# kutieme/avenir

Measured on AMD Instinct MI355X. Metric: naive_bayes_train_rows_per_s, higher is better.
Workload: dtype row-packed categorical records (11-bit records, lossless)/int64 counts (exact); 1 GPU; model=NaiveBayes(resource/churn.json: 5 categorical features, 2 classes), global_batch=1073741824, rows_per_gpu=1073741824, parallelism=dp1

## Files before the change

### avenir_amd/csrc/bindings.cpp

```cpp
#include <atomic>
#include <cstdlib>
#include <condition_variable>
#include <cstring>
#include <functional>
#include <chrono>
#include <limits>
#include <map>
#include <memory>
#include <mutex>
#include <thread>
#include <unistd.h>
#include <sys/stat.h>
#include <sys/mman.h>
#include <fcntl.h>
#include <torch/extension.h>
#include <ATen/hip/impl/HIPGuardImplMasqueradingAsCUDA.h>
#include <ATen/hip/impl/HIPStreamMasqueradingAsCUDA.h>

#include "avenir_kernels.h"
#include "avenir_host.h"

namespace {

using DevGuard = c10::hip::HIPGuardMasqueradingAsCUDA;
// ... 139 lines not shown
    TORCH_CHECK(widths[k] >= 1 && widths[k] <= 8 && shifts[k] >= 0 && shifts[k] + widths[k] <= B,
                "packed field outside the record");
    sh[k] = (int)shifts[k];
    wd[k] = (int)widths[k];
  }
  TORCH_CHECK(n_classes >= 1 && n_classes <= 2, "1 or 2 classes");
  CHECK_DEV(bins); CHECK_DTYPE(bins, at::kInt);
  CHECK_DEV(offs); CHECK_DTYPE(offs, at::kInt);
  TORCH_CHECK(bins.numel() == F && offs.numel() == F, "bins / offs must have F entries");
  TORCH_CHECK((int64_t)bins_host.size() == F && (int64_t)offs_host.size() == F, "bins_host / offs_host: F entries");
  for (int64_t k = 0; k < F; ++k)
    TORCH_CHECK(offs_host[k] >= 0 && bins_host[k] >= 1 && offs_host[k] + bins_host[k] <= total_bins,
                "feature bins outside the table");
  CHECK_DEV(out); CHECK_DTYPE(out, at::kLong);
  TORCH_CHECK(out.numel() == n_classes * total_bins, "out must be [C * TB]");
  DevGuard g(dense.device());
  avk::class_histogram_dense(reinterpret_cast<const uint32_t*>(dense.data_ptr<int>()), n, (int)B, sh.data(), wd.data(),
                             (int)F, (int)label_shift, (int)label_width, bins.data_ptr<int>(), offs.data_ptr<int>(),
                             (int)total_bins, (int)n_classes, count_labels ? 1 : 0,
                             reinterpret_cast<unsigned long long*>(out.data_ptr<int64_t>()), cur_stream(dense));
}

static std::vector<int> radix_ints(const std::vector<int64_t>& v, int64_t F, const char* what) {
  TORCH_CHECK((int64_t)v.size() == F, what, ": F entries");
  std::vector<int> r(F);
  for (int64_t k = 0; k < F; ++k) {
    TORCH_CHECK(v[k] >= 0 && v[k] < (int64_t(1) << 30), what, " out of range");
    r[k] = (int)v[k];
  }
  return r;
}

std::vector<int64_t> radix_shape(std::vector<int64_t> radices, int64_t class_radix, int64_t n_classes,
                                 int64_t total_bins) {
  TORCH_CHECK(class_radix >= 1 && class_radix <= 3 && n_classes >= 1 && n_classes <= 2 && total_bins >= 0 &&
                  total_bins < (int64_t(1) << 24), "bad class radix / classes / table width");
  int64_t J = class_radix;
  for (int64_t r : radices) {
    TORCH_CHECK(r >= 1 && r <= 9, "radix out of range");
    J *= r;
    TORCH_CHECK(J <= (int64_t(1) << 40), "too many joint states");
  }
  return {J, (int64_t)avk::radix_bits(J), (int64_t)avk::radix_replicas(J, (int)n_classes, (int)total_bins)};
}

at::Tensor pack_radix(const at::Tensor& words, int64_t n, int64_t B, std::vector<int64_t> shifts,
                      std::vector<int64_t> widths, std::vector<int64_t> radices, std::vector<int64_t> bins_host,
                      int64_t label_shift, int64_t class_radix, int64_t n_classes) {
  CHECK_DEV(words);
  CHECK_DTYPE(words, at::kShort);
  TORCH_CHECK(words.dim() == 1 && n >= 0 && n <= words.numel(), "words must be [>= n]");
  TORCH_CHECK(B >= 4 && B <= 15, "4..15 bits per record");
  const int64_t F = (int64_t)shifts.size();
  TORCH_CHECK(F >= 1 && F <= 8, "1..8 packed fields");
  const auto sh = radix_ints(shifts, F, "shifts"), wd = radix_ints(widths, F, "widths");
  const auto rad = radix_ints(radices, F, "radices"), hb = radix_ints(bins_host, F, "bins");
  auto dense = at::zeros({std::max<int64_t>(1, avk::dense_words(n, (int)B))}, words.options().dtype(at::kInt));
  DevGuard g(words.device());
  avk::pack_radix(reinterpret_cast<const uint16_t*>(words.data_ptr()), n, (int)B, sh.data(), wd.data(), rad.data(),
                  hb.data(), (int)F, (int)label_shift, (int)class_radix, (int)n_classes,
                  reinterpret_cast<uint32_t*>(dense.data_ptr<int>()), cur_stream(words));
  return dense;
}

void class_histogram_radix(const at::Tensor& dense, int64_t n, int64_t B, std::vector<int64_t> radices,
                           std::vector<int64_t> bins_host, std::vector<int64_t> offs_host, int64_t class_radix,
                           int64_t total_bins, int64_t n_classes, at::Tensor& out, bool count_labels) {
  CHECK_DEV(dense);
  CHECK_DTYPE(dense, at::kInt);
  TORCH_CHECK(B >= 4 && B <= 15 && n >= 0 && dense.numel() >= avk::dense_words(n, (int)B), "radix stream too short");
  const int64_t F = (int64_t)radices.size();
  TORCH_CHECK(F >= 1 && F <= 8, "1..8 packed fields");
  const auto rad = radix_ints(radices, F, "radices"), hb = radix_ints(bins_host, F, "bins");
  const auto ho = radix_ints(offs_host, F, "offs");
  TORCH_CHECK(n_classes >= 1 && n_classes <= 2, "1 or 2 classes");
  TORCH_CHECK(total_bins >= 1 && total_bins < (int64_t(1) << 24), "bad table width");
  CHECK_DEV(out); CHECK_DTYPE(out, at::kLong);
  TORCH_CHECK(out.numel() == n_classes * total_bins, "out must be [C * TB]");
  DevGuard g(dense.device());
  avk::class_histogram_radix(reinterpret_cast<const uint32_t*>(dense.data_ptr<int>()), n, (int)B, rad.data(), hb.data(),
                             ho.data(), (int)F, (int)class_radix, (int)total_bins, (int)n_classes,
                             count_labels ? 1 : 0, reinterpret_cast<unsigned long long*>(out.data_ptr<int64_t>()),
                             cur_stream(dense));
}

void pair_histogram(const at::Tensor& codes, int64_t n, const c10::optional<at::Tensor>& labels,
                    const at::Tensor& bins, const at::Tensor& pairs, const at::Tensor& poff,
                    int64_t max_tab, int64_t n_classes, at::Tensor& out) {
  CHECK_DEV(codes);
  CHECK_DTYPE(codes, at::kByte);
  TORCH_CHECK(codes.dim() == 2 && n <= codes.size(1), "codes must be [F, ld>=n]");
  CHECK_DEV(bins);
  CHECK_DTYPE(bins, at::kInt);
  CHECK_DEV(pairs);
  CHECK_DTYPE(pairs, at::kInt);
  CHECK_DEV(poff);
  CHECK_DTYPE(poff, at::kLong);
  CHECK_DEV(out);
  CHECK_DTYPE(out, at::kLong);
  TORCH_CHECK(pairs.dim() == 2 && pairs.size(1) == 2, "pairs must be [P,2]");
  TORCH_CHECK(poff.numel() == pairs.size(0), "poff must be [P]");
  const uint8_t* lab = nullptr;
  if (labels.has_value() && labels->defined()) {
    CHECK_DEV((*labels));
    CHECK_DTYPE((*labels), at::kByte);
    TORCH_CHECK(labels->numel() >= n, "labels shorter than n");
    lab = labels->data_ptr<uint8_t>();
  }
  DevGuard g(codes.device());
  avk::pair_histogram(codes.data_ptr<uint8_t>(), codes.size(1), n, lab, bins.data_ptr<int>(),
                      pairs.data_ptr<int>(), reinterpret_cast<const long long*>(poff.data_ptr<int64_t>()), (int)pairs.size(0),
                      (int)max_tab, (int)n_classes,
                      reinterpret_cast<unsigned long long*>(out.data_ptr<int64_t>()),
                      cur_stream(codes));
}

void bigram_histogram(const at::Tensor& states, const c10::optional<at::Tensor>& labels,
                      int64_t n_classes, int64_t S, at::Tensor& out) {
  CHECK_DEV(states);
  CHECK_DTYPE(states, at::kShort);
  TORCH_CHECK(states.dim() == 2, "states must be [N, L]");
  CHECK_DEV(out);
  CHECK_DTYPE(out, at::kLong);
  TORCH_CHECK(out.numel() == n_classes * S * S, "out must be [C*S*S]");
  TORCH_CHECK(S >= 1 && S <= 32767, "bad S");
  const uint8_t* lab = nullptr;
  if (labels.has_value() && labels->defined()) {
    CHECK_DEV((*labels));
    CHECK_DTYPE((*labels), at::kByte);
    TORCH_CHECK(labels->numel() >= states.size(0), "labels shorter than N");
    lab = labels->data_ptr<uint8_t>();
  }
  DevGuard g(states.device());
  avk::bigram_histogram(states.data_ptr<int16_t>(), states.size(0), (int)states.size(1), lab,
                        (int)n_classes, (int)S,
                        reinterpret_cast<unsigned long long*>(out.data_ptr<int64_t>()),
                        cur_stream(states));
}

at::Tensor class_moments(const at::Tensor& x, int64_t n, const c10::optional<at::Tensor>& labels,
                         int64_t n_classes) {
  CHECK_DEV(x);
  CHECK_DTYPE(x, at::kFloat);
  TORCH_CHECK(x.dim() == 2 && n <= x.size(1), "x must be [F, ld>=n]");
  const uint8_t* lab = nullptr;
  if (labels.has_value() && labels->defined()) {
    CHECK_DEV((*labels));
    CHECK_DTYPE((*labels), at::kByte);
    TORCH_CHECK(labels->numel() >= n, "labels shorter than n");
    lab = labels->data_ptr<uint8_t>();
  }
  const int64_t F = x.size(0);
  DevGuard g(x.device());
  auto opts = x.options().dtype(at::kDouble);
  auto out = at::zeros({n_classes, F, 3}, opts);
  const int nb = avk::moments_blocks(n);
  auto part = at::empty({nb, n_classes, F, 3}, opts);
  avk::class_moments(x.data_ptr<float>(), x.size(1), n, (int)F, lab, (int)n_classes,
                     part.data_ptr<double>(), nb, out.data_ptr<double>(), cur_stream(x));
  return out;
}

void nb_predict(const at::Tensor& codes, int64_t n, const at::Tensor& offs, const at::Tensor& logp,
                const c10::optional<at::Tensor>& logfp, const c10::optional<at::Tensor>& x,
                const c10::optional<at::Tensor>& gmean, const c10::optional<at::Tensor>& ginvstd,
                const c10::optional<at::Tensor>& glognorm, const c10::optional<at::Tensor>& pmean,
// ... 3555 lines not shown
                    training ? gates.data_ptr<float>() : nullptr, training ? hx.data_ptr<float>() : nullptr,
                    cur_stream(wfrag));
  if (training) return {hseq, cseq, gates, hx};
  return {hseq, cseq};
}

std::vector<at::Tensor> lstm_backward_f32(const at::Tensor& dhseq, const at::Tensor& gates, const at::Tensor& cseq,
                                          const c10::optional<at::Tensor>& c0, const c10::optional<at::Tensor>& dhn,
                                          const c10::optional<at::Tensor>& dcn, const at::Tensor& wfragT, int64_t H) {
  const int64_t KS = lstm_ks(H), HP = 32 * KS;
  for (const at::Tensor* t : std::initializer_list<const at::Tensor*>{&dhseq, &gates, &cseq, &wfragT}) {
    CHECK_DEV((*t));
    CHECK_DTYPE((*t), at::kFloat);
    TORCH_CHECK(t->is_contiguous() && aligned(*t, 16), "LSTM backward inputs must be contiguous and 16-byte aligned");
  }
  TORCH_CHECK(dhseq.dim() == 3 && dhseq.size(2) == H, "dhseq must be [B, T, H]");
  const int64_t B = dhseq.size(0), T = dhseq.size(1);
  TORCH_CHECK(cseq.dim() == 3 && cseq.size(0) == B && cseq.size(1) == T && cseq.size(2) == HP,
              "cseq must be [B, T, HP]");
  TORCH_CHECK(gates.dim() == 3 && gates.size(0) == B && gates.size(1) == T && gates.size(2) == 4 * HP,
              "gates must be [B, T, 4HP]");
  TORCH_CHECK(wfragT.numel() == 2 * KS * HP * 64, "wfragT must be [NW, HP, 64]");
  check_opt_f32(c0, B * H, "c0");
  check_opt_f32(dhn, B * H, "dhn");
  check_opt_f32(dcn, B * H, "dcn");
  DevGuard g(dhseq.device());
  auto dz = at::empty({B, T, 4 * H}, dhseq.options());
  auto dh0 = at::empty({B, H}, dhseq.options()), dc0 = at::empty({B, H}, dhseq.options());
  avk::lstm_bwd_f32(dhseq.data_ptr<float>(), gates.data_ptr<float>(), cseq.data_ptr<float>(), ptr_or_null<float>(c0),
                    ptr_or_null<float>(dhn), ptr_or_null<float>(dcn), wfragT.data_ptr<float>(), (int)B, (int)T, (int)H,
                    (int)KS, dz.data_ptr<float>(), dh0.data_ptr<float>(), dc0.data_ptr<float>(), cur_stream(dhseq));
  return {dz, dh0, dc0};
}

std::vector<at::Tensor> lstm_backward(const at::Tensor& dhseq, const at::Tensor& gates, const at::Tensor& cseq,
                                      const c10::optional<at::Tensor>& c0, const c10::optional<at::Tensor>& dhn,
                                      const c10::optional<at::Tensor>& dcn, const at::Tensor& wfragT, int64_t H) {
  const int64_t KS = lstm_ks(H), HP = 32 * KS;
  for (const at::Tensor* t : std::initializer_list<const at::Tensor*>{&dhseq, &gates, &cseq}) {
    CHECK_DEV((*t));
    CHECK_DTYPE((*t), t == &gates ? at::kBFloat16 : at::kFloat);
    TORCH_CHECK(aligned(*t, 16), "LSTM backward inputs must be 16-byte aligned");
  }
  TORCH_CHECK(dhseq.dim() == 3 && dhseq.size(2) == H, "dhseq must be [B, T, H]");
  const int64_t B = dhseq.size(0), T = dhseq.size(1);
  TORCH_CHECK(cseq.dim() == 3 && cseq.size(0) == B && cseq.size(1) == T && cseq.size(2) == HP,
              "cseq must be [B, T, HP]");
  TORCH_CHECK(gates.dim() == 3 && gates.size(0) == B && gates.size(1) == T && gates.size(2) == 4 * HP,
              "gates must be [B, T, 4HP]");
  CHECK_DEV(wfragT);
  CHECK_DTYPE(wfragT, at::kBFloat16);
  TORCH_CHECK(wfragT.numel() == 2 * KS * 4 * KS * 64 * 8, "wfragT must be [NW, 4KS, 64, 8]");
  TORCH_CHECK(aligned(wfragT, 16), "wfragT must be 16-byte aligned");
  check_opt_f32(c0, B * H, "c0");
  check_opt_f32(dhn, B * H, "dhn");
  check_opt_f32(dcn, B * H, "dcn");
  DevGuard g(dhseq.device());
  auto dz = at::empty({B, T, 4 * HP}, dhseq.options().dtype(at::kBFloat16));
  auto dh0 = at::empty({B, H}, dhseq.options()), dc0 = at::empty({B, H}, dhseq.options());
  const int RT = avk::lstm_row_tiles(B, (int)KS);
  avk::lstm_bwd(dhseq.data_ptr<float>(), reinterpret_cast<const unsigned short*>(gates.data_ptr()),
                cseq.data_ptr<float>(), ptr_or_null<float>(c0), ptr_or_null<float>(dhn), ptr_or_null<float>(dcn),
                wfragT.data_ptr(), (int)B, (int)T, (int)H, (int)KS, RT,
                reinterpret_cast<unsigned short*>(dz.data_ptr()), dh0.data_ptr<float>(), dc0.data_ptr<float>(),
                cur_stream(dhseq));
  return {dz, dh0, dc0};
}

}

void register_comm(py::module_& m);

PYBIND11_MODULE(_C, m) {
  register_comm(m);
  m.doc() = "avenir_amd native kernels (HIP/CDNA4 gfx950) and host runtime";
  m.def("class_histogram", &class_histogram);
  m.def("pair_histogram", &pair_histogram);
  m.def("class_histogram_rowpacked", &class_histogram_rowpacked);
  m.def("pack_dense", &pack_dense);
  m.def("class_histogram_dense", &class_histogram_dense);
  m.def("radix_shape", &radix_shape);
  m.def("pack_radix", &pack_radix);
  m.def("class_histogram_radix", &class_histogram_radix);
  m.def("bigram_histogram", &bigram_histogram);
  m.def("class_moments", &class_moments);
  m.def("nb_predict", &nb_predict);
  m.def("nb_predict_wide", &nb_predict_wide);
  m.def("node_histogram", &node_histogram, py::arg("codes"), py::arg("n"), py::arg("labels"), py::arg("node"),
        py::arg("weight"), py::arg("bins"), py::arg("offs"), py::arg("total_bins"), py::arg("n_classes"),
        py::arg("n_nodes"), py::arg("hist"), py::arg("node_rows") = py::none());
  m.def("node_grad_histogram", &node_grad_histogram, py::arg("codes"), py::arg("n"), py::arg("node"), py::arg("g"),
        py::arg("h"), py::arg("bins"), py::arg("offs"), py::arg("total_bins"), py::arg("n_nodes"), py::arg("out"),
        py::arg("even_only") = false, py::arg("tot_slot") = -1, py::arg("scale") = 65536.0);
  m.def("gbt_grad", &gbt_grad);
  m.def("gbt_split", &gbt_split);
  m.def("rank_avg", &rank_avg);
  m.def("tfidf_csr", &tfidf_csr);
  m.def("mixed_knn", &mixed_knn);
  m.def("pagerank", &pagerank);
  m.def("pagerank_multi", &pagerank_multi);
  m.def("sgns_hot_replicas", &avk::sgns_hot_replicas);
  m.def("sgns_step", &sgns_step, py::arg("Win"), py::arg("Wout"), py::arg("gIn"), py::arg("gOut"), py::arg("cIn"),
        py::arg("cOut"), py::arg("centre"), py::arg("context"), py::arg("aprob"), py::arg("alias"), py::arg("neg"),
        py::arg("lr"), py::arg("mean_in"), py::arg("seed"), py::arg("step"), py::arg("hot") = py::none(),
        py::arg("gOutHot") = py::none(), py::arg("gInHot") = py::none(), py::arg("cIn_next") = py::none(),
        py::arg("cOut_next") = py::none());
  m.def("kendall_pairs", &kendall_pairs);
  m.def("inversion_count", &inversion_count);
  m.def("resample_uniform", &resample_uniform);
  m.def("smote", &smote);
  m.def("gbt_assign", &gbt_assign);
  m.def("tree_assign", &tree_assign);
  m.def("tree_predict", &tree_predict);
  m.def("knn_topk", &knn_topk, py::arg("Q"), py::arg("R"), py::arg("k"), py::arg("q_base"), py::arg("r_base"),
        py::arg("exclude_self"), py::arg("splits"), py::arg("metric"), py::arg("p"), py::arg("prec") = -1);
  m.def("knn_mode", &avk::knn_mode);
  m.def("knn_vote", &knn_vote);
  m.def("cluster_accumulate", &cluster_accumulate);
  m.def("viterbi", &viterbi);
  m.def("viterbi_chunks", &viterbi_chunks);
  m.def("viterbi_backtrack", &viterbi_backtrack);
  m.def("markov_logodds", &markov_logodds);
  m.def("itemset_support", &itemset_support);
  m.def("build_bitsets", &build_bitsets);
  m.def("bandit_select", &bandit_select);
  m.def("sample", &sample);
  m.def("philox_normal", [](int64_t seed, int64_t offset, int64_t index_base, int64_t n, bool pairs,
                            c10::optional<at::Device> device) {
    TORCH_CHECK(n >= 0 && index_base >= 0, "philox_normal: n, index_base >= 0");
    if (device.has_value() && device->is_cuda()) {
      auto out = pairs ? at::empty({n, 2}, at::TensorOptions().dtype(at::kDouble).device(*device))
                       : at::empty({n}, at::TensorOptions().dtype(at::kDouble).device(*device));
      DevGuard g(*device);
      avk::philox_normal((unsigned long long)seed, (unsigned long long)offset, (unsigned long long)index_base, n,
                         out.data_ptr<double>(), pairs ? 1 : 0, cur_stream(out));
      return out;
    }
    auto out = pairs ? at::empty({n, 2}, at::TensorOptions().dtype(at::kDouble))
                     : at::empty({n}, at::TensorOptions().dtype(at::kDouble));
    {
      py::gil_scoped_release nogil;
      const unsigned hc = std::thread::hardware_concurrency();
      avh::philox_normal((uint64_t)seed, (uint64_t)offset, (uint64_t)index_base, n, out.data_ptr<double>(),
                         (int)std::min(16u, hc ? hc : 4u), pairs ? 1 : 0);
    }
    return out;
  }, "N(0,1) draws of Philox(seed, offset, index_base + i), host, fp64 (pairs: both Box-Muller outputs)",
        py::arg("seed"), py::arg("offset"), py::arg("index_base"), py::arg("n"), py::arg("pairs") = false,
        py::arg("device") = py::none());
  m.def("sa_assign", &sa_assign);
  m.def("ga_assign", &ga_assign);
  m.def("ga_assign_lds", [](int64_t P, int64_t L, int64_t r) { return (int64_t)avk::ga_assign_lds((int)P, (int)L, (int)r); });
  m.def("ga_meeting", &ga_meeting);
  m.def("ga_meeting_lds", [](int64_t P, int64_t L, int64_t r) { return (int64_t)avk::ga_meeting_lds((int)P, (int)L, (int)r); });
  m.def("smote_lines", &smote_lines);
  m.def("format_device", &format_device);
  m.def("pairs_within", &pairs_within);
  m.def("mixed_knn_max_dims", []() { return avk::mixed_knn_max_dims(); });
  m.def("glm_gradient", &glm_gradient);
  m.def("smo_solve", &smo_solve);
  m.def("smo_ws_solve", &smo_ws_solve);
  m.def("smo_ws_select", &smo_ws_select);
  m.def("smo_ws_update", &smo_ws_update);
  m.def("smo_ws_run", &smo_ws_run);
  m.def("smo_ws_run_x", &smo_ws_run_x, py::arg("X"), py::arg("xn"), py::arg("kind"), py::arg("gamma"),
        py::arg("coef0"), py::arg("degree"), py::arg("alpha"), py::arg("G"), py::arg("y"), py::arg("C"), py::arg("eps"),
// ... 162 lines not shown
```

### avenir_amd/csrc/include/avenir_kernels.h

```cpp
#pragma once
#include <hip/hip_runtime.h>
#include <stdint.h>
#include <algorithm>
#include <stdexcept>

namespace avk {

void class_histogram(const uint8_t* codes, long long ld, long long n, const uint8_t* labels,
                     const int* d_bins, const int* d_offs, const int* h_bins, int nfeat,
                     int total_bins, int n_classes, int count_labels, unsigned long long* out,
                     int mode, hipStream_t stream);
void class_histogram_wide(const uint16_t* codes, long long ld, long long n, const uint8_t* labels, const int* d_bins,
                          const int* d_offs, int nfeat, int total_bins, int n_classes, int count_labels,
                          unsigned long long* out, int mode, hipStream_t stream);
void class_histogram_i32(const int* codes, long long ld, long long n, const uint8_t* labels, const int* d_bins,
                          const int* d_offs, int nfeat, int total_bins, int n_classes, int count_labels,
                          unsigned long long* out, int mode, hipStream_t stream);
void pair_histogram(const uint8_t* codes, long long ld, long long n, const uint8_t* labels,
                    const int* d_bins, const int* d_pairs, const long long* d_poff, int n_pairs,
                    int max_tab, int n_classes, unsigned long long* out, hipStream_t stream);
void bigram_histogram(const int16_t* states, long long n, int L, const uint8_t* labels,
                      int n_classes, int S, unsigned long long* out, hipStream_t stream);
void class_moments(const float* x, long long ld, long long n, int nfeat, const uint8_t* labels,
                   int n_classes, double* part, int nblocks, double* out, hipStream_t stream);
// ... 167 lines not shown
void gemm_tn(const float* A, const float* B, float* C, float* partial, int K, int M, int N, int S, hipStream_t stream,
             int prec = -1);
int gemm_tn_mode();

void lstm_fwd_f32(const float* xw, const float* x, const float* wxfrag, const float* biask, const float* wfrag,
                  const float* h0, const float* c0, int B, int T, int H, int I, int KS, float* hseq, float* cseq,
                  float* gates, float* hx, hipStream_t s);
void lstm_pack_f32(const float* w_ih, const float* w_hh, const float* b_ih, const float* b_hh, int H, int I, int KS,
                   float* wfrag, float* wfragT, float* wihk, float* biask, float* wxfrag, hipStream_t s);
void lstm_bwd_f32(const float* dhseq, const float* gates, const float* cseq, const float* c0, const float* dhn,
                  const float* dcn, const float* wfragT, int B, int T, int H, int KS, float* dz, float* dh0,
                  float* dc0, hipStream_t s);

void nb_finalize(const long long* counts, int C, int TB, const int* offs, const int* bins, int F, float laplace,
                 float log_floor, float* logp, float* logfp, float* logprior, hipStream_t stream);

int gram_grid(long long n);
void weighted_gram(const float* X, long long ld, long long n, int D, const float* h, float* partial, int grid,
                   hipStream_t stream);

int kmeans_grid(long long n, int D, int K, int R);
void kmeans_assign(const float* X, long long n, int D, const float* C2, const float* Cn, const int* roff, int R, int K,
                   int* assign, float* partial, double* sse_partial, int grid, hipStream_t stream);
void kmeans_reduce(const float* partial, const double* sse_partial, int grid, int K, int D, int R, double* out,
                   hipStream_t stream);
void kmeans_update(const double* flat, int K, int D, int R, const int* run_of, const unsigned char* frozen, float* C2,
                   float* Cn, float* moves, hipStream_t stream);

void ngram_count(const short* st, long long n, int L, int S, int min_len, int max_len, const int* group,
                 unsigned long long group_mul, unsigned long long* keys, unsigned* counts, unsigned long long cap,
                 int* overflow, hipStream_t stream);
void hash_compact(const unsigned long long* keys, const unsigned* counts, unsigned long long cap, long long* out_keys,
                  long long* out_counts, unsigned long long* n_out, hipStream_t stream);
void uniformization(const double* P, int S, const double* w1, const double* w2, const int* steps, int ldw, int B,
                    double* out, hipStream_t stream);
void dot_matrix(const int* A, int n, int Wa, const int* B, int m, int Wb, int* hits, hipStream_t stream);

void bucketize_u8(const float* X, long long ldx, long long n, int F, const float* edges, const int* eoff, uint8_t* out,
                  long long ldo, hipStream_t stream);
void forest_hist(const uint8_t* codes, long long ld, const uint8_t* lab, const uint8_t* wt, const int* item_slot,
                 const long long* item_start, const int* item_len, int n_items, const int* bins, const int* offs,
                 int nfeat, int TB, int C, unsigned long long* hist, hipStream_t stream);
void forest_split(const long long* hist, const uint8_t* fmask, const int* bins, const int* offs, int nfeat, int TB,
                  int C, int algo, int topk, const float* rnd, int A, int* feat, int* thr, float* score, float* imp,
                  long long* left, hipStream_t stream);
void forest_part_count(const uint8_t* codes, long long ld, const int* item_node, const long long* item_start,
                       const int* item_len, int n_items, const int* feat, const int* thr, int* item_left,
                       hipStream_t stream);
int linear_act_fwd_slices(int M, int N, int K);
int f32_gemm_mode();
int linear_splitk_partial(const float* X, const float* W, float* partial, int M, int N, int K, int S,
                          hipStream_t stream, int prec = -1);
long long linear_act_fwd_planes_bytes(int M, int N, int K, int prec = -1);
long long sbf16_weight_planes_bytes(int N, int K, int prec = -1);
void sbf16_weight_planes(const float* W, int N, int K, int prec, void* out, hipStream_t stream);
void linear_act_fwd(const float* X, const float* W, const float* b, float* Y, int M, int N, int K, int act,
                    hipStream_t stream, float* partial = nullptr, int S = 1, int prec = -1, void* planes = nullptr,
                    const void* w_planes = nullptr);
int linear_act_bwd_rows(int M, int N);
int linear_act_bwd_blocks(int M, int N);
void linear_act_bwd(const float* dY, const float* Y, float* dZ, float* partial, int M, int N, int act,
                    hipStream_t stream);
int linear_act_wgrad_slices(int M, int N, int K);
void linear_act_wgrad(const float* dY, const float* Y, const float* X, float* dZ, float* pW, float* tmp, float* out,
                      int M, int N, int K, int act, hipStream_t stream);
long long forest_predict_bin_lds(int n_nodes, int nfeat);
void forest_predict_bin(const uint8_t* codes, long long ld, long long n, int nfeat, const uint2* nodes, int n_nodes,
                        const float* values, int V, const int* tree_root, const float* tree_w, int n_trees, int mode,
                        float* out, hipStream_t stream);
long long dense_words(long long n, int B);
void pack_dense(const uint16_t* words, long long n, int B, uint32_t* dense, hipStream_t stream);
void class_histogram_dense(const uint32_t* dense, long long n, int B, const int* h_shift, const int* h_width,
                           int nfeat, int label_shift, int label_width, const int* d_bins, const int* d_offs,
                           int total_bins, int n_classes, int count_labels, unsigned long long* out,
                           hipStream_t stream);
int radix_bits(long long J);
int radix_replicas(long long J, int n_classes, int total_bins);
void pack_radix(const uint16_t* words, long long n, int B, const int* h_shift, const int* h_width, const int* h_radix,
                const int* h_bins, int nfeat, int label_shift, int class_radix, int n_classes, uint32_t* dense,
                hipStream_t stream);
void class_histogram_radix(const uint32_t* dense, long long n, int B, const int* h_radix, const int* h_bins,
                           const int* h_offs, int nfeat, int class_radix, int total_bins, int n_classes,
                           int count_labels, unsigned long long* out, hipStream_t stream);
long long csv_chunks(long long size);
unsigned long long csv_slow_tokens_take(hipStream_t stream);
unsigned long long rec_slow_tokens_take(hipStream_t stream);
void csv_newline_counts(const uint8_t* bytes, long long size, unsigned* counts, hipStream_t stream);
void csv_newline_positions(const uint8_t* bytes, long long size, const long long* offsets, long long* pos,
                           hipStream_t stream);
void csv_line_bounds(const uint8_t* bytes, const long long* pos, long long nl, long long* starts, long long* ends,
                     uint8_t* keep, unsigned long long* blank, hipStream_t stream);
void csv_parse_rows(const uint8_t* bytes, long long size_padded, const long long* starts, const long long* ends,
                    long long n, char delim, const void* specs, int nspecs, int max_ord, const int* tabs,
                    const int* voff, const int* vlen, const uint8_t* vbytes, int ntab, int nvoc, int nvb,
                    unsigned long long* short_rows, hipStream_t stream);
int csv_devspec_bytes();
void resample_uniform(unsigned long long seed, unsigned long long stream, long long base, long long n, float* out,
                      hipStream_t st);
void smote(const float* X, const float* Xn, const int* nn, const int* Cs, const int* Cn, long long m, int k, int D,
           int Dc, int mult, long long gbase, unsigned long long seed, int exponential, float exp_mean, float* outX,
           int* outC, int* outPick, hipStream_t st);
void gbt_grad(const float* F, int K, int k, const uint8_t* y, long long n, long long row_off, unsigned long long seed,
              unsigned rate32, float* g, float* h, double* loss, hipStream_t stream);
void gbt_split(const long long* hist, const long long* parent, const long long* left, long long* out_hist, int A,
               int TB, int tot, const int* pfeat, const int* pthr, const int* pstart, const int* pend,
               const unsigned char* pvalid, int nb, double l2, double invS, int hb, int hc, int level0, int* feat,
               int* thr, double* val, hipStream_t stream);
void gbt_assign(const uint8_t* codes, long long ld, long long n, int* node, const int* feat, const int* thr,
                const double* value, const int* bins, int level, int last, float lr, float* F, int K, int k,
                hipStream_t stream);
void rec_lines(const uint8_t* bytes, const long long* nlpos, long long nraw, const char* delims, int ndelims,
               long long* lstart, long long* lend, int* ntok, hipStream_t stream);
void rec_tokens(const uint8_t* bytes, const long long* lstart, const long long* lend, const long long* off, long long L,
                const char* delims, int ndelims, const char* modes, int nmodes, char tail_mode, char sub_delim,
                bool trim, char last_mode, unsigned long long* keys, unsigned* h2tab, unsigned long long* first,
                unsigned long long mask, int* tslot, unsigned* th2, int* tsub, unsigned* th2sub, double* nums,
                unsigned* inserted, unsigned* overflow, hipStream_t stream);
void rec_codes(const int* tslot, const unsigned* th2, long long T, const int* slot_code, const unsigned* h2tab,
               int* codes, unsigned* mismatch, hipStream_t stream);
void rec_vocab(const uint8_t* bytes, const long long* lstart, const long long* lend, const long long* off, long long L,
               const unsigned long long* occ, long long D, const char* delims, int ndelims, char sub_delim, bool trim,
               long long* vstart, int* vlen, hipStream_t stream);
void rec_gather(const uint8_t* bytes, const long long* vstart, const int* vlen, const long long* vout, long long D,
                uint8_t* out, hipStream_t stream);
void forest_boot_count(const unsigned long long* keys, int ntrees, long long n, long long row_off, int mode,
                       unsigned rate32, int* tile_cnt, hipStream_t stream);
void forest_boot_scatter(const uint8_t* codes, long long ld, int nfeat, const uint8_t* lab,
                         const unsigned long long* keys, int ntrees, long long n, long long row_off, int mode,
                         unsigned rate32, const long long* tile_off, uint8_t* dcodes, uint8_t* dlab, uint8_t* dwt,
                         long long ldb, hipStream_t stream);
void forest_part_scatter(const uint8_t* codes, const uint8_t* lab, const uint8_t* wt, uint8_t* dcodes, uint8_t* dlab,
                         uint8_t* dwt, long long ld, int nfeat, const int* item_node, const long long* item_start,
                         const int* item_len, int n_items, const long long* left_base, const long long* right_base,
                         const int* feat, const int* thr, hipStream_t stream);

void gsp_count(const int* X, int N, int k, int lo, int hi, int* seg_start, int* seg_len, hipStream_t stream);
void gsp_emit(const int* X, int k, int lo, int hi, const int* seg_start, const int* seg_len, const long long* offs,
              int* out, hipStream_t stream);

int col_moments_blocks(long long n, int F);
void col_moments_f32(const float* X, long long n, long long ld, int F, int pass, const double* mean, double* part,
                     hipStream_t stream);
void col_moments_f64(const double* X, long long n, long long ld, int F, int pass, const double* mean, double* part,
                     hipStream_t stream);
void loo_stats(const void* codes, int code_bytes, int m, long long ld, long long n, int F, const double* y, double* sum,
               unsigned* cnt, hipStream_t stream);
void loo_apply(const void* codes, int code_bytes, int m, long long ld, long long n, int F, const double* y, const double* sum,
               const unsigned* cnt, const double* gmean, double reg, const double* noise, double amp, float* out,
               hipStream_t stream);

void spirit_update(const double* X, int K, int T, int D, int H, const int* lens, double* W, double* E, double* he,
                   double* ve, double* cnt, int* nh, double lam, double lo, double hi, hipStream_t stream);

int lstm_row_tiles(long long B, int KS);
void lstm_fwd(const float* x, int I, int IS, const void* wfrag, const float* bias, const float* h0, const float* c0,
              int B, int T, int H, int KS, int RT, float* hseq, float* cseq, unsigned short* gates, unsigned short* hx,
              hipStream_t stream);
void lstm_bwd(const float* dhseq, const unsigned short* gates, const float* cseq, const float* c0, const float* dhn,
              const float* dcn, const void* wfragT, int B, int T, int H, int KS, int RT, unsigned short* dz,
              float* dh0, float* dc0, hipStream_t stream);

int mixed_knn_max_dims();
int mixed_knn_splits(long long nq, long long nr);
void mixed_knn(const float* Qn, const int* Qc, long long nq, const float* Rn, const int* Rc, long long nr, int Dn,
               int Dc, const float* wc, int k, long long r_base, float* out_d, long long* out_i, float* part_d,
               int* part_i, int splits, hipStream_t stream);
// ... 71 lines not shown
```

### avenir_amd/csrc/kernels/histogram.hip

```cpp
#include <cstdlib>
#include <string>

#include "avenir_common.h"
#include "avenir_kernels.h"

namespace {

constexpr int HB = 256;
constexpr int FLUSH_EVERY = 15;

__device__ __forceinline__ void flush_packed(unsigned long long& lo, unsigned long long& hi,
                                             unsigned int* s_bins ) {
  const unsigned long long M = 0x00FF00FF00FF00FFull;
  unsigned long long w[4] = {lo & M, (lo >> 8) & M, hi & M, (hi >> 8) & M};
#pragma unroll
  for (int q = 0; q < 4; ++q) w[q] = av::wave_sum_u64(w[q]);
  if (av::lane_id() == 0) {
#pragma unroll
    for (int q = 0; q < 4; ++q) {
      const int base = (q >> 1) * 8 + (q & 1);
#pragma unroll
      for (int k = 0; k < 4; ++k) {
        unsigned v = (unsigned)((w[q] >> (16 * k)) & 0xFFFFu);
        if (v) atomicAdd(&s_bins[base + 2 * k], v);
// ... 569 lines not shown
    const uint32_t* src = dense + g * B;
#pragma unroll
    for (int i = 0; i < B; ++i) d[i] = src[i];
    d[B] = 0;
    const long long left = n - (g << 5);
    auto rec = [&](int k) __attribute__((always_inline)) -> unsigned {
      const int bit = k * B, i = bit >> 5, sh = bit & 31;
      if (sh + B <= 32) return __builtin_amdgcn_ubfe(d[i], (unsigned)sh, (unsigned)B);
      return __builtin_amdgcn_alignbit(d[i + 1], d[i], (unsigned)sh) & M;
    };
    if (left >= 32) {
#pragma unroll
      for (int k = 0; k < 32; ++k) {
        const unsigned r = rec(k);
        atomicAdd(&s_joint[(r ^ (r >> S)) * R + rep], 1u);
      }
    } else {
#pragma unroll
      for (int k = 0; k < 32; ++k)
        if (k < left) {
        const unsigned r = rec(k);
        atomicAdd(&s_joint[(r ^ (r >> S)) * R + rep], 1u);
      }
    }
  }
  __syncthreads();
  for (int p = threadIdx.x; p < J; p += NT) {
    unsigned cnt = 0;
#pragma unroll
    for (int r = 0; r < R; ++r) cnt += s_joint[p * R + r];
    if (!cnt) continue;
    unsigned ju = (unsigned)p;
#pragma unroll
    for (int t = S; t < B; t += S) ju ^= (unsigned)p >> t;
    const int j = (int)ju;
    int c = 0;
    if (n_classes > 1) {
      const unsigned lb = __builtin_amdgcn_ubfe((unsigned)j, (unsigned)spec.lsh, (unsigned)n_classes);
      if (lb == 1u) c = 0;
      else if (lb == 2u) c = 1;
      else continue;
    }
    unsigned int* row = s_small + c * total_bins;
    for (int kf = 0; kf < nfeat; ++kf) {
      const int code = (int)__builtin_amdgcn_ubfe((unsigned)j, (unsigned)spec.sh[kf], (unsigned)spec.w[kf]);
      if (code < bins[kf]) atomicAdd(&row[offs[kf] + code], cnt);
    }
    if (count_labels) atomicAdd(&row[total_bins - 1], cnt);
  }
  __syncthreads();
  for (int i = threadIdx.x; i < n_classes * total_bins; i += NT) {
    const unsigned cnt = s_small[i];
    if (cnt) atomicAdd(&out[i], (unsigned long long)cnt);
  }
}

__global__ __launch_bounds__(HB) void pack_dense_kernel(const uint16_t* __restrict__ words, long long n, int B,
                                                        uint32_t* __restrict__ dense) {
  const long long groups = (n + 31) >> 5;
  const long long stride = (long long)gridDim.x * HB;
  for (long long g = (long long)blockIdx.x * HB + threadIdx.x; g < groups; g += stride) {
    uint32_t d[16];
#pragma unroll
    for (int i = 0; i < 16; ++i) d[i] = 0;
    for (int k = 0; k < 32; ++k) {
      const long long r = (g << 5) + k;
      const uint32_t v = r < n ? ((uint32_t)words[r] & ((1u << B) - 1u)) : 0u;
      const int bit = k * B, i = bit >> 5, sh = bit & 31;
#pragma unroll
      for (int q = 0; q < 16; ++q) {
        if (q == i) d[q] |= v << sh;
        if (q == i + 1 && sh + B > 32) d[q] |= v >> (32 - sh);
      }
    }
    for (int i = 0; i < B; ++i) dense[g * B + i] = d[i];
  }
}

struct RadixSpec {
  int rad[8];
  int bins[8];
  int offs[8];
  int crad;
};

__global__ __launch_bounds__(HB) void pack_radix_kernel(const uint16_t* __restrict__ words, long long n, int B,
                                                        RowPackSpec spec, RadixSpec rs, int nfeat,
                                                        uint32_t* __restrict__ dense) {
  const long long groups = (n + 31) >> 5;
  const long long stride = (long long)gridDim.x * HB;
  for (long long g = (long long)blockIdx.x * HB + threadIdx.x; g < groups; g += stride) {
    uint32_t d[16];
#pragma unroll
    for (int i = 0; i < 16; ++i) d[i] = 0;
    for (int k = 0; k < 32; ++k) {
      const long long r = (g << 5) + k;
      uint32_t v = 0;
      if (r < n) {
        const uint32_t w = words[r];
        uint32_t mult = 1;
        if (rs.crad > 1) {
          const uint32_t lb = __builtin_amdgcn_ubfe(w, (unsigned)spec.lsh, 2u);
          const uint32_t cd = lb == 1u ? 0u : (lb == 2u ? 1u : 2u);
          v = min(cd, (uint32_t)rs.crad - 1u);
          mult = (uint32_t)rs.crad;
        }
        for (int f = 0; f < nfeat; ++f) {
          const uint32_t code = __builtin_amdgcn_ubfe(w, (unsigned)spec.sh[f], (unsigned)spec.w[f]);
          v += min(code, (uint32_t)rs.rad[f] - 1u) * mult;
          mult *= (uint32_t)rs.rad[f];
        }
      }
      const int bit = k * B, i = bit >> 5, sh = bit & 31;
#pragma unroll
      for (int q = 0; q < 16; ++q) {
        if (q == i) d[q] |= v << sh;
        if (q == i + 1 && sh + B > 32) d[q] |= v >> (32 - sh);
      }
    }
    for (int i = 0; i < B; ++i) dense[g * B + i] = d[i];
  }
}

template <int B>
__global__ __launch_bounds__(1024) void hist_joint_radix_kernel(const uint32_t* __restrict__ dense, long long n,
                                                                RadixSpec rs, int J, int log2r, int nfeat,
                                                                int n_classes, int total_bins, int count_labels,
                                                                unsigned long long* __restrict__ out) {
  extern __shared__ __attribute__((aligned(16))) unsigned int s_joint[];
  constexpr unsigned M = (1u << B) - 1u;
  const int NT = (int)blockDim.x;
  const int R = 1 << log2r;
  unsigned int* s_small = s_joint + ((size_t)J << log2r);
  for (int i = threadIdx.x; i < (J << log2r) + n_classes * total_bins; i += NT) s_joint[i] = 0;
  char* const my = reinterpret_cast<char*>(s_joint + (threadIdx.x & (unsigned)(R - 1)));
  const unsigned lr = (unsigned)log2r + 2u;
  __syncthreads();
  const long long groups = (n + 31) >> 5;
  const long long stride = (long long)gridDim.x * NT;
  for (long long g = (long long)blockIdx.x * NT + threadIdx.x; g < groups; g += stride) {
    uint32_t d[B + 1];
    const uint32_t* src = dense + g * B;
#pragma unroll
    for (int i = 0; i < B; ++i) d[i] = src[i];
    d[B] = 0;
    const long long left = n - (g << 5);
    auto rec = [&](int k) __attribute__((always_inline)) -> unsigned {
      const int bit = k * B, i = bit >> 5, sh = bit & 31;
      if (sh + B <= 32) return __builtin_amdgcn_ubfe(d[i], (unsigned)sh, (unsigned)B);
      return __builtin_amdgcn_alignbit(d[i + 1], d[i], (unsigned)sh) & M;
    };
    if (left >= 32) {
#pragma unroll
      for (int k = 0; k < 32; ++k) atomicAdd(reinterpret_cast<unsigned int*>(my + (rec(k) << lr)), 1u);
    } else {
#pragma unroll
      for (int k = 0; k < 32; ++k)
        if (k < left) atomicAdd(reinterpret_cast<unsigned int*>(my + (rec(k) << lr)), 1u);
    }
  }
  __syncthreads();
  const int ls = log2r < 3 ? log2r : 3;
  const int S = 1 << ls;
  const int items = J << ls;
  for (int base = 0; base < items; base += NT) {
    const int i = base + (int)threadIdx.x;
    const int cell = i >> ls;
    unsigned cnt = 0;
    if (i < items)
      for (int q = 0; q < (R >> ls); ++q) cnt += s_joint[((size_t)cell << log2r) + ((i + (q << ls)) & (R - 1))];
    for (int o = S >> 1; o; o >>= 1) cnt += __shfl_xor(cnt, o);
    unsigned j = (unsigned)cell;
    int c = 0;
    if (rs.crad > 1) {
      c = (int)(j % (unsigned)rs.crad);
      j /= (unsigned)rs.crad;
    }
    if (i < items && !(i & (S - 1)) && cnt && c < n_classes) {
      unsigned int* row = s_small + c * total_bins;
      for (int kf = 0; kf < nfeat; ++kf) {
        const unsigned rk = (unsigned)rs.rad[kf];
        const int code = (int)(j % rk);
        j /= rk;
        if (code < rs.bins[kf]) atomicAdd(&row[rs.offs[kf] + code], cnt);
      }
      if (count_labels) atomicAdd(&row[total_bins - 1], cnt);
    }
  }
  __syncthreads();
  for (int i = threadIdx.x; i < n_classes * total_bins; i += NT) {
    const unsigned cnt = s_small[i];
    if (cnt) atomicAdd(&out[i], (unsigned long long)cnt);
  }
}

int hist_joint_lds(int nbits, int n_classes, int total_bins) {
  return (int)(sizeof(unsigned) * ((size_t(1) << nbits) + (size_t)n_classes * total_bins));
}

struct RowPackLaunch {
  const uint16_t* words;
  long long n;
  RowPackSpec spec;
  const int* bins;
  const int* offs;
  int total_bins, count_labels;
  unsigned long long* out;
  hipStream_t stream;
};

template <int NF, int C, int NM>
void launch_rowpack(const RowPackLaunch& a) {
  static const int res = av::resident_blocks((const void*)hist_rowpack_kernel<NF, C, NM>, HB, 0);
  const int grid = std::min(av::stream_grid(std::max(1LL, a.n >> 3), HB, 4, 4096), res);
  hist_rowpack_kernel<NF, C, NM><<<grid, HB, 0, a.stream>>>(a.words, a.n, a.spec, a.bins, a.offs, a.total_bins,
                                                            a.count_labels, a.out);
  AV_HIP_CHECK(hipGetLastError());
}

template <int NF, int NM>
void launch_rowpack_c2(int nm, const RowPackLaunch& a) {
  if constexpr (NM > NF) {
    throw std::runtime_error("row-packed histogram: bad merged-feature count");
  } else {
    if (nm == NM) launch_rowpack<NF, 2, NM>(a);
    else launch_rowpack_c2<NF, NM + 1>(nm, a);
  }
}

template <int NF>
void launch_rowpack_nf(int n_classes, int nm, const RowPackLaunch& a) {
  if (n_classes == 1) launch_rowpack<NF, 1, 0>(a);
  else launch_rowpack_c2<NF, 0>(nm, a);
}

__global__ __launch_bounds__(HB) void hist_lds_kernel(
    const uint8_t* __restrict__ codes, long long ld, long long n, const uint8_t* __restrict__ labels,
    const int* __restrict__ bins, const int* __restrict__ offs, int nfeat, int total_bins,
    int n_classes, int count_labels, int replicas, unsigned long long* __restrict__ out) {
  extern __shared__ __attribute__((aligned(16))) unsigned int s_tab[];
  const int tab = n_classes * total_bins;
  for (int i = threadIdx.x; i < tab * replicas; i += HB) s_tab[i] = 0;
  __syncthreads();
  unsigned int* my = s_tab + (av::wave_id() % replicas) * tab;
  const long long stride = (long long)gridDim.x * HB;
  for (long long r = (long long)blockIdx.x * HB + threadIdx.x; r < n; r += stride) {
    const unsigned c = labels ? labels[r] : 0u;
    if (c >= (unsigned)n_classes) continue;
    for (int f = 0; f < nfeat; ++f) {
      const unsigned v = codes[(long long)f * ld + r];
      if (v < (unsigned)bins[f]) atomicAdd(&my[c * total_bins + offs[f] + v], 1u);
    }
    if (count_labels) atomicAdd(&my[c * total_bins + total_bins - 1], 1u);
  }
  __syncthreads();
  for (int i = threadIdx.x; i < tab; i += HB) {
    unsigned long long s = 0;
    for (int q = 0; q < replicas; ++q) s += s_tab[q * tab + i];
    if (s) atomicAdd(&out[i], s);
  }
}

__global__ __launch_bounds__(HB) void hist_global_kernel(
    const uint8_t* __restrict__ codes, long long ld, long long n, const uint8_t* __restrict__ labels,
    const int* __restrict__ bins, const int* __restrict__ offs, int nfeat, int total_bins,
    int n_classes, int count_labels, unsigned long long* __restrict__ out) {
  const long long stride = (long long)gridDim.x * HB;
  for (long long r = (long long)blockIdx.x * HB + threadIdx.x; r < n; r += stride) {
    const unsigned c = labels ? labels[r] : 0u;
    if (c >= (unsigned)n_classes) continue;
    for (int f = 0; f < nfeat; ++f) {
      const unsigned v = codes[(long long)f * ld + r];
      if (v < (unsigned)bins[f])
// ... 270 lines not shown
  }
  const RowPackLaunch a{words, n, spec, d_bins, d_offs, total_bins, count_labels, out, stream};
  switch (nfeat) {
    case 1: launch_rowpack_nf<1>(n_classes, nm, a); break;
    case 2: launch_rowpack_nf<2>(n_classes, nm, a); break;
    case 3: launch_rowpack_nf<3>(n_classes, nm, a); break;
    case 4: launch_rowpack_nf<4>(n_classes, nm, a); break;
    case 5: launch_rowpack_nf<5>(n_classes, nm, a); break;
    case 6: launch_rowpack_nf<6>(n_classes, nm, a); break;
    case 7: launch_rowpack_nf<7>(n_classes, nm, a); break;
    default: launch_rowpack_nf<8>(n_classes, nm, a); break;
  }
}


long long dense_words(long long n, int B) { return ((n + 31) >> 5) * (long long)B; }

void pack_dense(const uint16_t* words, long long n, int B, uint32_t* dense, hipStream_t stream) {
  if (n <= 0) return;
  if (B < 1 || B > 15) throw std::runtime_error("pack_dense: 1..15 bits per record");
  pack_dense_kernel<<<av::stream_grid((n + 31) >> 5, HB, 1, 4096), HB, 0, stream>>>(words, n, B, dense);
  AV_HIP_CHECK(hipGetLastError());
}

template <int B, int R, int NT>
static void launch_joint_dense_r(const uint32_t* dense, long long n, const RowPackSpec& spec, int nfeat, int n_classes,
                                 const int* bins, const int* offs, int total_bins, int count_labels,
                                 unsigned long long* out, hipStream_t stream) {
  const int lds = (int)(sizeof(unsigned) * ((size_t)R * (size_t(1) << B) + (size_t)n_classes * total_bins));
  if (lds > 160 * 1024) throw std::runtime_error("dense histogram: replicated table exceeds LDS");
  auto kern = hist_joint_dense_kernel<B, R, NT>;
  if (lds > 64 * 1024)
    AV_HIP_CHECK(hipFuncSetAttribute(reinterpret_cast<const void*>(kern), hipFuncAttributeMaxDynamicSharedMemorySize,
                                     lds));
  const int res = av::resident_blocks((const void*)kern, NT, (size_t)lds);
  const int grid = std::max(1, std::min(av::stream_grid(std::max(1LL, (n + 31) >> 5), NT, 1, 8192), res));
  kern<<<grid, NT, (size_t)lds, stream>>>(dense, n, spec, nfeat, n_classes, bins, offs, total_bins, count_labels, out);
  AV_HIP_CHECK(hipGetLastError());
}

template <int B>
static void launch_joint_dense(const uint32_t* dense, long long n, const RowPackSpec& spec, int nfeat, int n_classes,
                               const int* bins, const int* offs, int total_bins, int count_labels,
                               unsigned long long* out, hipStream_t stream) {
  int R = (B <= 13) ? 4 : (B == 14 ? 2 : 1);
  if (const char* e = std::getenv("AVMI_JOINT_REPLICAS")) R = std::atoi(e);
  if (R >= 4 && B <= 13)
    launch_joint_dense_r<B, 4, 1024>(dense, n, spec, nfeat, n_classes, bins, offs, total_bins, count_labels, out, stream);
  else if (R >= 2 && B <= 14)
    launch_joint_dense_r<B, 2, 512>(dense, n, spec, nfeat, n_classes, bins, offs, total_bins, count_labels, out, stream);
  else
    launch_joint_dense_r<B, 1, HB>(dense, n, spec, nfeat, n_classes, bins, offs, total_bins, count_labels, out, stream);
}

void class_histogram_dense(const uint32_t* dense, long long n, int B, const int* h_shift, const int* h_width,
                           int nfeat, int label_shift, int label_width, const int* d_bins, const int* d_offs,
                           int total_bins, int n_classes, int count_labels, unsigned long long* out,
                           hipStream_t stream) {
  if (n <= 0 || nfeat <= 0) return;
  if (nfeat > 8 || n_classes < 1 || n_classes > 2) throw std::runtime_error("dense histogram: F <= 8, C <= 2");
  if (n_classes > 1 && (label_width != n_classes || label_shift != 0))
    throw std::runtime_error("dense histogram: the class is C one-hot bits at bit 0");
  RowPackSpec spec{};
  int need = n_classes > 1 ? label_width : 1;
  for (int k = 0; k < nfeat; ++k) {
    spec.sh[k] = h_shift[k];
    spec.w[k] = h_width[k];
    need = std::max(need, h_shift[k] + h_width[k]);
  }
  spec.lsh = n_classes > 1 ? label_shift : 0;
  if (need > B) throw std::runtime_error("dense histogram: fields exceed the record width");
  switch (B) {
#define AV_DENSE(BB) \
  case BB: launch_joint_dense<BB>(dense, n, spec, nfeat, n_classes, d_bins, d_offs, total_bins, count_labels, out, stream); break;
    AV_DENSE(4) AV_DENSE(5) AV_DENSE(6) AV_DENSE(7) AV_DENSE(8) AV_DENSE(9) AV_DENSE(10) AV_DENSE(11)
    AV_DENSE(12) AV_DENSE(13) AV_DENSE(14) AV_DENSE(15)
#undef AV_DENSE
    default: throw std::runtime_error("dense histogram: 4..15 bits per record");
  }
}

constexpr int kLdsPerCu = 160 * 1024;

static RadixSpec radix_spec(const int* h_radix, const int* h_bins, const int* h_offs, int nfeat, int class_radix,
                            int n_classes, int total_bins, long long* J) {
  if (nfeat < 1 || nfeat > 8 || n_classes < 1 || n_classes > 2)
    throw std::runtime_error("radix histogram: 1 <= F <= 8, C <= 2");
  if (n_classes == 1 ? class_radix != 1 : (class_radix != 2 && class_radix != 3))
    throw std::runtime_error("radix histogram: class radix 1 (C = 1), 2 or 3 (C = 2)");
  RadixSpec rs{};
  rs.crad = class_radix;
  long long j = class_radix;
  for (int k = 0; k < nfeat; ++k) {
    if (h_bins[k] < 1 || (h_radix[k] != h_bins[k] && h_radix[k] != h_bins[k] + 1))
      throw std::runtime_error("radix histogram: a radix is bins or bins + 1");
    if (h_offs[k] < 0 || h_offs[k] + h_bins[k] > total_bins)
      throw std::runtime_error("radix histogram: feature bins outside the table");
    rs.rad[k] = h_radix[k];
    rs.bins[k] = h_bins[k];
    rs.offs[k] = h_offs[k];
    j *= h_radix[k];
    if (j > (1LL << 15)) throw std::runtime_error("radix histogram: more than 2^15 joint states");
  }
  *J = j;
  return rs;
}

int radix_bits(long long J) {
  int b = 0;
  while ((1LL << b) < J) ++b;
  return b;
}

void pack_radix(const uint16_t* words, long long n, int B, const int* h_shift, const int* h_width, const int* h_radix,
                const int* h_bins, int nfeat, int label_shift, int class_radix, int n_classes, uint32_t* dense,
                hipStream_t stream) {
  if (n <= 0) return;
  const int offs0[8] = {0, 0, 0, 0, 0, 0, 0, 0};
  long long J = 0;
  const RadixSpec rs = radix_spec(h_radix, h_bins, offs0, nfeat, class_radix, n_classes, 1 << 30, &J);
  if (B < 4 || B > 15 || radix_bits(J) != B) throw std::runtime_error("pack_radix: B = ceil(log2 J) in 4..15");
  RowPackSpec spec{};
  for (int k = 0; k < nfeat; ++k) {
    if (h_width[k] < 1 || h_width[k] > 3 || h_shift[k] < 0 || h_shift[k] + h_width[k] > 16)
      throw std::runtime_error("pack_radix: fields of 1..3 bits inside the 16-bit word");
    spec.sh[k] = h_shift[k];
    spec.w[k] = h_width[k];
  }
  if (n_classes > 1 && (label_shift < 0 || label_shift + 2 > 16))
    throw std::runtime_error("pack_radix: the class is two one-hot bits inside the 16-bit word");
  spec.lsh = n_classes > 1 ? label_shift : 0;
  pack_radix_kernel<<<av::stream_grid((n + 31) >> 5, HB, 1, 4096), HB, 0, stream>>>(words, n, B, spec, rs, nfeat, dense);
  AV_HIP_CHECK(hipGetLastError());
}

int radix_replicas(long long J, int n_classes, int total_bins) {
  int want = 32;
  if (const char* e = std::getenv("AVMI_JOINT_REPLICAS")) want = std::max(1, std::min(32, std::atoi(e)));
  int R = 1;
  while (R * 2 <= want && 4LL * (J * (R * 2) + (long long)n_classes * total_bins) <= kLdsPerCu) R *= 2;
  return R;
}

template <int B>
static void launch_joint_radix(const uint32_t* dense, long long n, const RadixSpec& rs, int J, int nfeat,
                               int n_classes, int total_bins, int count_labels, unsigned long long* out,
                               hipStream_t stream) {
  const int R = radix_replicas(J, n_classes, total_bins);
  const long long lds = 4LL * ((long long)J * R + (long long)n_classes * total_bins);
  if (lds > kLdsPerCu) throw std::runtime_error("radix histogram: joint table exceeds LDS");
  int log2r = 0;
  while ((1 << log2r) < R) ++log2r;
  const int per_cu = (int)(kLdsPerCu / lds);
  const int NT = per_cu >= 4 ? HB : (per_cu >= 2 ? 512 : 1024);
  auto kern = hist_joint_radix_kernel<B>;
  static int c_dev = -1, c_lds = -1, c_nt = 0, c_res = 0;
  int dev = 0;
  AV_HIP_CHECK(hipGetDevice(&dev));
  if (c_dev != dev || c_lds != (int)lds || c_nt != NT) {
    if (lds > 64 * 1024)
      AV_HIP_CHECK(hipFuncSetAttribute(reinterpret_cast<const void*>(kern), hipFuncAttributeMaxDynamicSharedMemorySize,
                                       (int)lds));
    c_res = av::resident_blocks((const void*)kern, NT, (size_t)lds);
    c_dev = dev;
    c_lds = (int)lds;
    c_nt = NT;
  }
  const int grid = std::max(1, std::min(av::stream_grid(std::max(1LL, (n + 31) >> 5), NT, 1, 8192), c_res));
  kern<<<grid, NT, (size_t)lds, stream>>>(dense, n, rs, J, log2r, nfeat, n_classes, total_bins, count_labels, out);
  AV_HIP_CHECK(hipGetLastError());
}

void class_histogram_radix(const uint32_t* dense, long long n, int B, const int* h_radix, const int* h_bins,
                           const int* h_offs, int nfeat, int class_radix, int total_bins, int n_classes,
                           int count_labels, unsigned long long* out, hipStream_t stream) {
  if (n <= 0) return;
  long long J = 0;
  const RadixSpec rs = radix_spec(h_radix, h_bins, h_offs, nfeat, class_radix, n_classes, total_bins, &J);
  if (radix_bits(J) != B) throw std::runtime_error("radix histogram: B = ceil(log2 J)");
  if (count_labels && total_bins < 1) throw std::runtime_error("radix histogram: no class-count column");
  switch (B) {
#define AV_RADIX(BB) \
  case BB: launch_joint_radix<BB>(dense, n, rs, (int)J, nfeat, n_classes, total_bins, count_labels, out, stream); break;
// ... 9 lines not shown
```

Measured before the change: 4136 billion rows/s.

## Prefetch next radix group and split joint-state decode across lanes with reciprocals

The radix histogram kernel now loads the next group's packed words before finishing the current one, so global loads overlap the LDS atomic work, and the first load is issued before the shared-memory clear. The joint-state reduction decodes per-feature codes with precomputed multiply-high reciprocals instead of integer division, and spreads the features of one cell across the S lanes that already hold the reduced count instead of having one lane loop over all features. This costs a few more registers and extra fields in the spec struct, and relies on the reciprocal trick being exact for divisors up to 2^15. A Python binding for the reciprocal is also exposed.

```diff
diff --git a/avenir_amd/csrc/bindings.cpp b/avenir_amd/csrc/bindings.cpp
--- a/avenir_amd/csrc/bindings.cpp
+++ b/avenir_amd/csrc/bindings.cpp
@@ -245,6 +245,11 @@
                              ho.data(), (int)F, (int)class_radix, (int)total_bins, (int)n_classes,
                              count_labels ? 1 : 0, reinterpret_cast<unsigned long long*>(out.data_ptr<int64_t>()),
                              cur_stream(dense));
+}
+
+int64_t radix_recip(int64_t d) {
+  TORCH_CHECK(d >= 1 && d <= (int64_t(1) << 15), "divisor out of range");
+  return (int64_t)avk::radix_recip((unsigned)d);
 }
 
 void pair_histogram(const at::Tensor& codes, int64_t n, const c10::optional<at::Tensor>& labels,
@@ -3966,6 +3971,7 @@
   m.def("radix_shape", &radix_shape);
   m.def("pack_radix", &pack_radix);
   m.def("class_histogram_radix", &class_histogram_radix);
+  m.def("radix_recip", &radix_recip);
   m.def("bigram_histogram", &bigram_histogram);
   m.def("class_moments", &class_moments);
   m.def("nb_predict", &nb_predict);
diff --git a/avenir_amd/csrc/include/avenir_kernels.h b/avenir_amd/csrc/include/avenir_kernels.h
--- a/avenir_amd/csrc/include/avenir_kernels.h
+++ b/avenir_amd/csrc/include/avenir_kernels.h
@@ -273,6 +273,7 @@
 void class_histogram_radix(const uint32_t* dense, long long n, int B, const int* h_radix, const int* h_bins,
                            const int* h_offs, int nfeat, int class_radix, int total_bins, int n_classes,
                            int count_labels, unsigned long long* out, hipStream_t stream);
+unsigned radix_recip(unsigned d);
 long long csv_chunks(long long size);
 unsigned long long csv_slow_tokens_take(hipStream_t stream);
 unsigned long long rec_slow_tokens_take(hipStream_t stream);
diff --git a/avenir_amd/csrc/kernels/histogram.hip b/avenir_amd/csrc/kernels/histogram.hip
--- a/avenir_amd/csrc/kernels/histogram.hip
+++ b/avenir_amd/csrc/kernels/histogram.hip
@@ -675,7 +675,12 @@
   int bins[8];
   int offs[8];
   int crad;
+  unsigned stride[8], srcp[8], rrcp[8], crcp;
 };
+
+__device__ __forceinline__ unsigned div_small(unsigned n, unsigned d, unsigned m) {
+  return d == 1u ? n : __umulhi(n, m);
+}
 
 __global__ __launch_bounds__(HB) void pack_radix_kernel(const uint16_t* __restrict__ words, long long n, int B,
                                                         RowPackSpec spec, RadixSpec rs, int nfeat,
@@ -724,19 +729,24 @@
   constexpr unsigned M = (1u << B) - 1u;
   const int NT = (int)blockDim.x;
   const int R = 1 << log2r;
+  const int ctb = n_classes * total_bins;
   unsigned int* s_small = s_joint + ((size_t)J << log2r);
-  for (int i = threadIdx.x; i < (J << log2r) + n_classes * total_bins; i += NT) s_joint[i] = 0;
+  const long long groups = (n + 31) >> 5;
+  const long long stride = (long long)gridDim.x * NT;
+  uint32_t d[B + 1];
+  d[B] = 0;
+  auto load = [&](long long g) __attribute__((always_inline)) {
+    const uint32_t* src = dense + g * B;
+#pragma unroll
+    for (int i = 0; i < B; ++i) d[i] = src[i];
+  };
+  long long g = (long long)blockIdx.x * NT + threadIdx.x;
+  if (g < groups) load(g);
+  for (int i = threadIdx.x; i < (J << log2r) + ctb; i += NT) s_joint[i] = 0;
   char* const my = reinterpret_cast<char*>(s_joint + (threadIdx.x & (unsigned)(R - 1)));
   const unsigned lr = (unsigned)log2r + 2u;
   __syncthreads();
-  const long long groups = (n + 31) >> 5;
-  const long long stride = (long long)gridDim.x * NT;
-  for (long long g = (long long)blockIdx.x * NT + threadIdx.x; g < groups; g += stride) {
-    uint32_t d[B + 1];
-    const uint32_t* src = dense + g * B;
-#pragma unroll
-    for (int i = 0; i < B; ++i) d[i] = src[i];
-    d[B] = 0;
+  while (g < groups) {
     const long long left = n - (g << 5);
     auto rec = [&](int k) __attribute__((always_inline)) -> unsigned {
       const int bit = k * B, i = bit >> 5, sh = bit & 31;
@@ -751,6 +761,8 @@
       for (int k = 0; k < 32; ++k)
         if (k < left) atomicAdd(reinterpret_cast<unsigned int*>(my + (rec(k) << lr)), 1u);
     }
+    g += stride;
+    if (g < groups) load(g);
   }
   __syncthreads();
   const int ls = log2r < 3 ? log2r : 3;
@@ -758,30 +770,27 @@
   const int items = J << ls;
   for (int base = 0; base < items; base += NT) {
     const int i = base + (int)threadIdx.x;
-    const int cell = i >> ls;
+    const unsigned cell = (unsigned)(i >> ls);
     unsigned cnt = 0;
     if (i < items)
       for (int q = 0; q < (R >> ls); ++q) cnt += s_joint[((size_t)cell << log2r) + ((i + (q << ls)) & (R - 1))];
     for (int o = S >> 1; o; o >>= 1) cnt += __shfl_xor(cnt, o);
-    unsigned j = (unsigned)cell;
-    int c = 0;
-    if (rs.crad > 1) {
-      c = (int)(j % (unsigned)rs.crad);
-      j /= (unsigned)rs.crad;
-    }
-    if (i < items && !(i & (S - 1)) && cnt && c < n_classes) {
+    const unsigned c = cell - div_small(cell, (unsigned)rs.crad, rs.crcp) * (unsigned)rs.crad;
+    if (i < items && cnt && c < (unsigned)n_classes) {
       unsigned int* row = s_small + c * total_bins;
-      for (int kf = 0; kf < nfeat; ++kf) {
-        const unsigned rk = (unsigned)rs.rad[kf];
-        const int code = (int)(j % rk);
-        j /= rk;
-        if (code < rs.bins[kf]) atomicAdd(&row[rs.offs[kf] + code], cnt);
-      }
-      if (count_labels) atomicAdd(&row[total_bins - 1], cnt);
-    }
-  }
-  __syncthreads();
-  for (int i = threadIdx.x; i < n_classes * total_bins; i += NT) {
+      for (int kf = i & (S - 1); kf <= nfeat; kf += S) {
+        if (kf == nfeat) {
+          if (count_labels) atomicAdd(&row[total_bins - 1], cnt);
+          break;
+        }
+        const unsigned q = div_small(cell, rs.stride[kf], rs.srcp[kf]), rk = (unsigned)rs.rad[kf];
+        const unsigned code = q - div_small(q, rk, rs.rrcp[kf]) * rk;
+        if (code < (unsigned)rs.bins[kf]) atomicAdd(&row[rs.offs[kf] + code], cnt);
+      }
+    }
+  }
+  __syncthreads();
+  for (int i = threadIdx.x; i < ctb; i += NT) {
     const unsigned cnt = s_small[i];
     if (cnt) atomicAdd(&out[i], (unsigned long long)cnt);
   }
@@ -1218,6 +1227,8 @@
 
 constexpr int kLdsPerCu = 160 * 1024;
 
+unsigned radix_recip(unsigned d) { return d < 2u ? 0u : (unsigned)((1ull << 32) / d + 1ull); }
+
 static RadixSpec radix_spec(const int* h_radix, const int* h_bins, const int* h_offs, int nfeat, int class_radix,
                             int n_classes, int total_bins, long long* J) {
   if (nfeat < 1 || nfeat > 8 || n_classes < 1 || n_classes > 2)
@@ -1226,6 +1237,7 @@
     throw std::runtime_error("radix histogram: class radix 1 (C = 1), 2 or 3 (C = 2)");
   RadixSpec rs{};
   rs.crad = class_radix;
+  rs.crcp = radix_recip((unsigned)class_radix);
   long long j = class_radix;
   for (int k = 0; k < nfeat; ++k) {
     if (h_bins[k] < 1 || (h_radix[k] != h_bins[k] && h_radix[k] != h_bins[k] + 1))
@@ -1235,6 +1247,9 @@
     rs.rad[k] = h_radix[k];
     rs.bins[k] = h_bins[k];
     rs.offs[k] = h_offs[k];
+    rs.stride[k] = (unsigned)j;
+    rs.srcp[k] = radix_recip((unsigned)j);
+    rs.rrcp[k] = radix_recip((unsigned)h_radix[k]);
     j *= h_radix[k];
     if (j > (1LL << 15)) throw std::runtime_error("radix histogram: more than 2^15 joint states");
   }
```

After: 4221 billion rows/s (median of 6 runs). 2.1% higher.
